# TMmichi/mujoco_jaco

Hardware: AMD Instinct MI355X
Metric: env-steps/sec at batch 65 536 (full Jaco + gripper + contacts) (higher is better)
Workload: dtype f32

## Files before the change

__graft_entry__.py:

```python
import os
import subprocess
import sys

ROOT = os.path.dirname(os.path.abspath(__file__))
CSRC = os.path.join(ROOT, "mujoco_jaco_amd", "csrc")
HIPCC = os.environ.get("HIPCC", "/opt/rocm/bin/hipcc")


D12 = ["-DJNB=13", "-DJNV=18", "-DJNQ=19", "-DJB0=12", "-DJB1=18", "-DJNSENS=64", "-DJMAXCHAIN=8", "-DJMAXDESC=12", "-DJMAXINNER=9"]
D30 = ["-DJNB=20", "-DJNV=30", "-DJNQ=32", "-DJB0=18", "-DJB1=24", "-DJNU=18", "-DJNSENS=40", "-DJMAXGEOM=128", "-DJMAXPAIR=3584", "-DJMAXINNER=12",
       "-DJMAXMPAIR=192", "-DJACO_LIGHT_WAVES=2"]


FLAGS = ["--offload-arch=gfx950", "-O3", "-std=c++17", "-fno-hip-fp32-correctly-rounded-divide-sqrt", "-fno-slp-vectorize",
         "-fgpu-flush-denormals-to-zero", "-fPIC", "-Rpass-analysis=kernel-resource-usage", "-I", os.path.join(CSRC, "include")]
NKERNEL_TU = 18


def _variant_jobs(name, extra):
    bdir = os.path.join(ROOT, "build", name)
    os.makedirs(bdir, exist_ok=True)
    jobs, objs = [], []
    for tu in list(range(NKERNEL_TU)) + [-1]:
        src = "jaco_env.hip" if tu < 0 else "kernels.hip"
# ... 15 lines not shown


def _up_to_date(cmd, log):
    obj, stamp = cmd[cmd.index("-o") + 1], log[:-4] + ".cmd"
    if not (os.path.exists(obj) and os.path.exists(stamp) and open(stamp).read() == " ".join(cmd)):
        return False
    t = os.path.getmtime(obj)
    return all(os.path.getmtime(d) < t for d in _sources_of(cmd))


def build_libs(variants, workers=None):
    workers = workers or max(1, min(8, os.cpu_count() or 1))
    todo, links = [], []
    for name, extra in variants.items():
        jobs, link = _variant_jobs(name, extra)
        jobs = [j for j in jobs if not _up_to_date(*j)]
        todo += sorted(jobs, key=lambda j: ("kernel7" in j[1], "kernel6" in j[1], "kernel5" in j[1], "kernel4" in j[1]), reverse=True)
        links.append(link)
    running, failed = [], []
    while todo or running:
        while todo and len(running) < workers and not failed:
            cmd, log = todo.pop(0)
            running.append((subprocess.Popen(cmd, cwd=CSRC, stdout=open(log, "w"), stderr=subprocess.STDOUT), cmd, log))
        if failed and not running:
            break
        p, cmd, log = running.pop(0)
        if p.poll() is None:
            running.append((p, cmd, log))
            import time
            time.sleep(0.2)
            continue
        if p.returncode == 0:
            open(log[:-4] + ".cmd", "w").write(" ".join(cmd))
        if p.returncode != 0:
            failed.append((cmd, log))
            for q, _, _ in running:
                q.terminate()
            for q, _, _ in running:
                q.wait()
            running = []
    if failed:
        cmd, log = failed[0]
        raise RuntimeError("hipcc failed: %s\n%s" % (" ".join(cmd), open(log).read()[-4000:]))
    for link in links:
        subprocess.check_call(link, cwd=CSRC)


VARIANTS = {
    "default": [],
    "d12": D12,
    "d30": D30,
    "prof": ["-DJACO_PROFILE_STAGES"],
    "noregime": ["-DJACO_NEWTON_REGIME=0"],
    "census": ["-DJACO_PROFILE_STAGES", "-DJACO_REGIME_CENSUS"],
}
PRODUCT = ("default", "d12", "d30")


def build():
    build_libs({k: v for k, v in VARIANTS.items() if k in PRODUCT or (k == "prof" and os.environ.get("JACO_BUILD_PROF") == "1")})
    subprocess.check_call(["make", "-s", "-C", os.path.join(ROOT, "oracle")])
    subprocess.check_call(["make", "-s", "-C", os.path.join(ROOT, "tests", "emu")])
    subprocess.check_call(["make", "-s", "-C", os.path.join(ROOT, "tests", "emu_lqr")])
    if os.path.isdir("/root/reference/env_script/assets/jaco2") and not os.path.exists(
            os.path.join(ROOT, "mujoco_jaco_amd", "assets", "jaco2_curtain_torque.jacomdl")):
        subprocess.check_call([sys.executable, "-m", "mujoco_jaco_amd.modelc.compile"], cwd=ROOT)
    sys.path.insert(0, ROOT)
    import mujoco_jaco_amd
    from mujoco_jaco_amd import _lib
    _lib.load()
    _lib.load("_d12")
    _lib.load("_d30")


def smoke():
    sys.path.insert(0, ROOT)
    sys.path.insert(0, os.path.join(ROOT, "tests"))
    import numpy as np
    import torch
    from mujoco_jaco_amd import workload
    from mujoco_jaco_amd.modelc import blob
    from mujoco_jaco_amd.physics import BatchedMujoco
    from oracle_binding import Oracle

    B, nsub = 64, 20
    M = blob.load(os.path.join(ROOT, "mujoco_jaco_amd", "assets", "jaco2_curtain_torque.jacomdl"))
    q = workload.reset_states(M["qpos0"], B, seed=7, f32_draws=True)
    c = workload.random_ctrl(B, seed=8, scale=0.2).astype(np.float32).astype(np.float64)
    env = BatchedMujoco(B, device=0)
    dev = env.device
    env.set_state(torch.tensor(q, dtype=torch.float32, device=dev), None, None)
    env.send_forces(torch.tensor(c, dtype=torch.float32, device=dev), nsub=nsub)
    gq, gv, _ = [t.cpu().numpy().astype(np.float64) for t in env.get_state()]
    o = Oracle()
    qo, vo, wo = q.copy(), np.zeros((B, 21)), np.zeros((B, 21))
    o.step_batch(qo, vo, wo, np.ascontiguousarray(c), nsub=nsub, nthreads=4)
    err = np.abs(gq - qo).max(axis=1)
    fl = env.flags().cpu().numpy()
    deepest = np.zeros(B)
    for k in range(B):
        o.set("qpos", q[k]); o.set("qvel", np.zeros(21)); o.forward()
        C = o.get("contact").reshape(-1, 11)
        deepest[k] = -C[:, 0].min() if len(C) else 0.0
    clean = deepest <= 0.0105
    print("smoke: %d envs x %d substeps on %s, qpos max-abs error vs fp64 oracle: median %.2e, p90 %.2e; max over the %d envs without deep start overlap %.2e, "
          "over the %d with it %.2e (deepest %.3f m); error flags %d, tiers used: %s"
# ... 16 lines not shown
```

mujoco_jaco_amd/csrc/collision.h:

```cpp
#pragma once

#define JACO_HAVE_COLLISION 1

struct GeomPose { v3 p; m3 R; };
template <class L>
JDEV GeomPose geom_pose(const L& s, int g) { GeomPose r; r.p = ld3(s.gpos[g]); r.R = ldm(s.gmat[g]); return r; }

JDEV bool obb_separated(const GeomPose& a, v3 sa, const GeomPose& b, v3 sb) {
  float C[3][3], Q[3][3];
  v3 d = b.p - a.p;
  float t[3] = {dot(d, col(a.R, 0)), dot(d, col(a.R, 1)), dot(d, col(a.R, 2))};
  float ea[3] = {sa.x, sa.y, sa.z}, eb[3] = {sb.x, sb.y, sb.z};
#pragma unroll
  for (int i = 0; i < 3; i++)
#pragma unroll
    for (int j = 0; j < 3; j++) { C[i][j] = dot(col(a.R, i), col(b.R, j)); Q[i][j] = fabsf(C[i][j]) + 1e-5f; }
  bool sep = false;
#pragma unroll
  for (int i = 0; i < 3; i++) sep |= fabsf(t[i]) > ea[i] + eb[0] * Q[i][0] + eb[1] * Q[i][1] + eb[2] * Q[i][2];
#pragma unroll
  for (int j = 0; j < 3; j++)
    sep |= fabsf(t[0] * C[0][j] + t[1] * C[1][j] + t[2] * C[2][j]) > eb[j] + ea[0] * Q[0][j] + ea[1] * Q[1][j] + ea[2] * Q[2][j];
#pragma unroll
  for (int i = 0; i < 3; i++)
// ... 884 lines not shown
      } else {
        float depth;
        v3 dir, pos;
#ifdef JACO_EMULATED
        const long q0_ = emu_counter[7];
#endif
        const MprGeom G1 = mpr_geom(m, s, g1, t1), G2 = mpr_geom(m, s, g2, t2);
#ifdef JACO_ROW_REUSE
        HullRow H1, H2;
        H1.cell = -1; H2.cell = -1; H1.e.x = H1.e.y = H1.e.z = H1.e.w = 0.f; H2.e = H1.e;
#endif
        const float sw = wave_bcast(sepA.w, c);
        bool hit = false, apart = false, sepvalid = false;
        v3 sep = mk3(0.f, 0.f, 0.f);
#if JACO_MPR_PAIRS
        if ((parked >> c) & 1ull) {
          const float* st = stash + 8 * c;
          hit = st[0] != 0.f; depth = st[1]; pos = mk3(st[2], st[3], st[4]); dir = mk3(st[5], st[6], st[7]);
          apart = true;
        } else
#endif
        if (sw != 0.f) {
          const v3 d = mk3(wave_bcast(sepA.x, c), wave_bcast(sepA.y, c), wave_bcast(sepA.z, c));
          const Sup q = mpr_support(A, G1, G2, d, lane JROWPASS);
          apart = dot(q.v, d) < -1e-5f && fabsf(dot(d, d) - 1.f) < 1e-3f;
        }
        if (!apart) {
          hit = mpr_penetration(A, m, G1, G2, lane, &depth, &dir, &pos, &sep, &sepvalid JROWPASS);
          if (seprow && lane == 0 && (sepvalid || sw != 0.f)) {
            v4 o; o.x = sep.x; o.y = sep.y; o.z = sep.z; o.w = sepvalid ? 1.f : 0.f;
            *reinterpret_cast<v4*>(seprow + 4 * pk) = o;
          }
        }
#ifdef JACO_EMULATED
        if (lane == 0 && !((parked >> c) & 1ull)) { emu_counter[3]++; emu_counter[4] += hit; emu_counter[hit ? 5 : 6] += emu_counter[7] - q0_; }
#endif
#ifdef JACO_TRACE_MPR
        if (lane == 0) printf("mpr g1 %d g2 %d hit %d depth %g\n", g1, g2, (int)hit, hit ? depth : 0.f);
#endif
        push_contacts(s, hit && lane == 0, -depth, pos, dir, pk, ncon, flags, 1);
        JSTAMP_NARROW(hit ? 14 : 1);
      }
      if (ncon > before) {
        int cc = before + lane;
        if (cc < ncon) { s.c_ob[cc] = pob; s.c_dim[cc] = pdim; }
      }
      c++;
    }
    if (L::Caps::MAXEFC < JacoHuge::MAXEFC && (wave_uniform_i((int)flags) & (int)JFLAG_CON_OVERFLOW)) break;
  }
  if (lane == 0) { s.ncon = ncon; s.ncand = ncand; }
}

#define JSIDE_ROWS 16
#define JSIDE_BASE 64
#define JSIDE_J 0
#define JSIDE_AREF 96
#define JSIDE_D 112
#define JSIDE_F 128
template <class L>
struct SideRows {
  static constexpr bool on = L::Caps::CONTACT && L::Caps::MAXEFC == 64 && JNV - JB1 == 6 && (JNV - 6) * 6 + JNB * 6 >= JSIDE_F + JSIDE_ROWS;
};
template <class L>
JDEV float* side_buf(L& s) { return &s.cdof[6][0]; }
template <class L>
JDEV float contact_row_vel(const L& s, int c, int e, float mu) {
  const int pd = s.c_dim[c];
  const int kf = pd == 1 ? 0 : 1 + (e >> 1);
  const int obs = s.c_ob[c], b1 = ((obs >> 8) & 0xFF) - 1, b2 = ((obs >> 24) & 0xFF) - 1;
  sv v1, v2;
  v1.a = v1.b = v2.a = v2.b = mk3(0.f, 0.f, 0.f);
  if (b1 >= 0) v1 = ldsv(s.cvel[b1]);
  if (b2 >= 0) v2 = ldsv(s.cvel[b2]);
  v3 cp = ld3(s.c_pos[c]);
  v3 dw = v2.a - v1.a, dv = (v2.b - v1.b) + cross(dw, cp);
  const float* fr = s.c_frame[c];
  float vel = dot(ld3(fr), dv);
  if (pd > 1) {
    const int ax = kf < 3 ? kf : kf - 3;
    const float comp = dot(ld3(fr + 3 * ax), kf < 3 ? dv : dw);
    vel += ((e & 1) ? -1.f : 1.f) * mu * comp;
  }
  return vel;
}
template <class L>
JDEV void stage_contact_rows(const JacoModelDev* m, L& s, int lane, unsigned& flags) {
  constexpr int MAXEFC = L::Caps::MAXEFC;
  constexpr bool SIDE = SideRows<L>::on;
  const int nv = m->nv, ncon = wave_uniform_i(s.ncon), nlim = wave_uniform_i(s.nlimit);
  float* sd = side_buf(s);
  int rowbase = nlim, kept_total = 0, nside = 0, side_cand = 0;
  constexpr int CPP = JNV <= 21 ? 3 : 64 / JNV;
  const int cl = lane / JNV, k = lane - cl * JNV;
  const bool dofok = cl < CPP && k < nv;
  const sv S = ldsv(s.cdof[dofok ? k : 0]);
  for (int cb = 0; cb < ncon; cb += 64) {
    const int ci = cb + lane, nhere = ncon - cb < 64 ? ncon - cb : 64;
    int dim = 0, nrow = 0;
    float mu0 = 0.f, mu1 = 0.f, mu2 = 0.f;
    unsigned cm1 = 0, cm2 = 0;
    float a0 = 0.f, bcoef = 0.f, dinv = 0.f;
    if (lane < nhere) {
      const JacoPairParam& P = m->pair[s.c_pair[ci]];
      dim = s.c_dim[ci]; nrow = dim == 1 ? 1 : 2 * (dim - 1);
      mu0 = P.mu[0]; mu1 = P.mu[2]; mu2 = P.mu[3];
      cm1 = P.m1; cm2 = P.m2;
      const float pos = s.c_dist[ci] - P.margin, tran = P.tran;
      float R, imp;
      a0 = row_params(P.solref, P.solimp, pos, 0.f, dim == 1 ? tran : tran + mu0 * mu0 * tran, &R, &imp);
      bcoef = 2.f / fmaxf(JMINVAL, fminf(0.9999f, fmaxf(0.0001f, P.solimp[1])) * P.solref[0]);
      if (dim > 1) R = fmaxf(JMINVAL, 2.f * mu0 * mu0 * R);
      dinv = 1.f / R;
    }
    const unsigned mm = cm1 | cm2;
    bool sidec = false;
    const unsigned long long upto = lane >= 63 ? ~0ull : ((2ull << lane) - 1ull);
    const unsigned long long r1m = wave_ballot(nrow == 1), r4m = wave_ballot(nrow == 4), r10m = wave_ballot(nrow == 10);
    const bool rows_std = wave_ballot(nrow != 0 && nrow != 1 && nrow != 4 && nrow != 10) == 0ull;
    int end = rowbase + (rows_std ? popc64(r1m & upto) + 4 * popc64(r4m & upto) + 10 * popc64(r10m & upto) : wave_scan_incl(nrow, lane));
#ifdef JACO_SIDE_ALWAYS
    if (JNV - JB1 == 6 && cb == 0) {
#else
    if (JNV - JB1 == 6 && cb == 0 && wave_bcast_i(end, nhere - 1) > JSIDE_BASE) {
#endif
      const bool only2 = lane < nhere && mm != 0u && (mm & ((1u << JB1) - 1u)) == 0u && nrow <= 4;
      const bool reach2 = lane < nhere && !only2 && (mm >> JB1) != 0u;
      const unsigned long long o2 = wave_ballot(only2);
      if (o2 != 0ull && wave_ballot(reach2) == 0ull && ncon <= 64) {
        int srows = 0;
        for (unsigned long long b = o2; b; b &= b - 1ull) srows += wave_bcast_i(nrow, ffs64(b));
        if (srows <= JSIDE_ROWS) { side_cand = srows; sidec = only2; }
      }
    }
    bool split = false;
    int r0s = 0;
#ifdef JACO_SIDE_ALWAYS
    if (SIDE && side_cand > 0 && wave_bcast_i(end, nhere - 1) - side_cand <= MAXEFC) {
#else
    if (SIDE && side_cand > 0 && wave_bcast_i(end, nhere - 1) > MAXEFC && wave_bcast_i(end, nhere - 1) - side_cand <= MAXEFC) {
#endif
      split = true;
      end = rowbase + wave_scan_incl(sidec ? 0 : nrow, lane);
      r0s = JSIDE_BASE + wave_scan_incl(sidec ? nrow : 0, lane) - nrow;
      nside = side_cand;
    }
    sidec = sidec && split;
    const unsigned long long fm = wave_ballot(lane < nhere && end <= MAXEFC);
    const int kept = popc64(fm);
    int total = wave_bcast_i(end, kept > 0 ? kept - 1 : 0);
    total = kept > 0 ? total : rowbase;
    const int r0 = sidec ? r0s : end - nrow;
    if (lane < kept) {
      s.c_efc[ci] = r0;
      int blk = ((mm & ((1u << JB0) - 1u)) ? 1 : 0) | (((mm >> JB0) & ((1u << (JB1 - JB0)) - 1u)) ? 2 : 0) | ((mm >> JB1) ? 4 : 0);
      const int bodies = L::Caps::WRENCH ? ((((s.c_ob[ci] >> 8) & 31) << 19) | (((s.c_ob[ci] >> 24) & 31) << 24)) : 0;
      if (!sidec) for (int e = 0; e < nrow; e++) {
        s.e_con[r0 + e] = ci | (e << 8) | (blk << 16) | bodies;
        s.e_f[r0 + e] = e < 4 ? mu0 : (e < 6 ? mu1 : mu2);
        s.e_aref[r0 + e] = a0; s.e_D[r0 + e] = dinv;
      }
      s.c_fn[ci] = bcoef;
    }
    wave_sync();
    for (int rr = rowbase + lane; rr < total; rr += 64) {
      const int ce = s.e_con[rr], c = ce & 255, e = (ce >> 8) & 255;
      const float vel = contact_row_vel(s, c, e, s.e_f[rr]);
      s.e_aref[rr] = s.e_aref[rr] - s.c_fn[c] * vel;
    }
    float aside[4] = {0.f, 0.f, 0.f, 0.f};
    if (SIDE && sidec && lane < kept) {
#pragma unroll
      for (int e = 0; e < 4; e++) if (e < nrow) aside[e] = a0 - bcoef * contact_row_vel(s, ci, e, mu0);
    }
    if (SIDE && split) {
      wave_sync();
      if (sidec && lane < kept) {
#pragma unroll
        for (int e = 0; e < 4; e++) if (e < nrow) { sd[JSIDE_AREF + r0 - JSIDE_BASE + e] = aside[e]; sd[JSIDE_D + r0 - JSIDE_BASE + e] = dinv; }
      }
    }
    if (L::Caps::WRENCH) {
      for (int rr = rowbase + lane; rr < total; rr += 64) {
        const int ce = s.e_con[rr], c = ce & 255, e = (ce >> 8) & 15, pd = s.c_dim[c];
        const int kf = pd == 1 ? 0 : 1 + (e >> 1);
        const float smu = ((e & 1) ? -1.f : 1.f) * s.e_f[rr];
        const float* fr = s.c_frame[c];
        const v3 n = ld3(fr), pos = ld3(s.c_pos[c]);
        v3 lin = n, ang = mk3(0.f, 0.f, 0.f);
        if (kf == 1 || kf == 2) lin = n + ld3(fr + 3 * kf) * smu;
        if (kf >= 3) ang = ld3(fr + 3 * (kf - 3)) * smu;
        ang = ang + cross(pos, lin);
        float* R = s.J + 8 * rr;
        R[0] = ang.x; R[1] = ang.y; R[2] = ang.z; R[3] = lin.x; R[4] = lin.y; R[5] = lin.z; R[6] = 0.f; R[7] = 0.f;
      }
    } else
    for (int c0 = 0; c0 < kept; c0 += CPP) {
      int c = c0 + (cl < CPP ? cl : 0);
      int src = c < 64 ? c : 0;
      int cdim = wave_shfl_i(dim, src), cr0 = wave_shfl_i(r0, src);
      float f0 = wave_shfl(mu0, src), f1 = wave_shfl(mu1, src), f2 = wave_shfl(mu2, src);
      unsigned a1 = (unsigned)wave_shfl_i((int)cm1, src), a2 = (unsigned)wave_shfl_i((int)cm2, src);
      const bool cside = SIDE && cr0 >= JSIDE_BASE;
      if (dofok && c < kept && (!cside || k >= JB1)) {
        float coef = (float)((int)((a2 >> k) & 1u) - (int)((a1 >> k) & 1u));
        v3 pos = ld3(s.c_pos[cb + c]);
        v3 jp = (S.b + cross(S.a, pos)) * coef, jr = S.a * coef;
        const float* fr = s.c_frame[cb + c];
        float Jc[6];
#pragma unroll
        for (int a = 0; a < 3; a++) { Jc[a] = dot(ld3(fr + 3 * a), jp); Jc[3 + a] = dot(ld3(fr + 3 * a), jr); }
        const int ld = cside ? 6 : JLD;
        float* Jw = cside ? sd + JSIDE_J + (cr0 - JSIDE_BASE) * 6 + (k - JB1) : s.J + cr0 * JLD + k;
        if (cdim == 1) Jw[0] = Jc[0];
        else {
          Jw[0] = Jc[0] + f0 * Jc[1]; Jw[ld] = Jc[0] - f0 * Jc[1];
          Jw[2 * ld] = Jc[0] + f0 * Jc[2]; Jw[3 * ld] = Jc[0] - f0 * Jc[2];
          if (cdim > 3) {
            Jw[4 * ld] = Jc[0] + f1 * Jc[3]; Jw[5 * ld] = Jc[0] - f1 * Jc[3];
            Jw[6 * ld] = Jc[0] + f2 * Jc[4]; Jw[7 * ld] = Jc[0] - f2 * Jc[4];
            Jw[8 * ld] = Jc[0] + f2 * Jc[5]; Jw[9 * ld] = Jc[0] - f2 * Jc[5];
          }
        }
      }
    }
    rowbase = total; kept_total += kept;
    if (kept < nhere) { flags |= JFLAG_EFC_OVERFLOW; break; }
  }
  const int total = rowbase;
  wave_sync();
  if (lane == 0) { s.nefc = total; s.ncon = kept_total; s.nside = nside; s.nside_cand = side_cand; }
}

JDEV bool ray_hits_site(int type, float sx, float sy, float sz, v3 p, v3 d) {
  sx += 1e-5f; sy += 1e-5f; sz += 1e-5f;
  float t0 = 0.f, t1 = 3.0e38f;
  bool ok = true;
  if (type == JG_BOX) {
    float pp[3] = {p.x, p.y, p.z}, dd[3] = {d.x, d.y, d.z}, ss[3] = {sx, sy, sz};
#pragma unroll
    for (int i = 0; i < 3; i++) {
      if (fabsf(dd[i]) < JMINVAL) { ok = ok && !(fabsf(pp[i]) > ss[i]); continue; }
      float a = (-ss[i] - pp[i]) / dd[i], b = (ss[i] - pp[i]) / dd[i];
      t0 = fmaxf(t0, fminf(a, b));
      t1 = fminf(t1, fmaxf(a, b));
    }
    return ok && t1 >= t0;
  }
  if (type == JG_CYLINDER) {
    if (fabsf(d.z) < JMINVAL) ok = !(fabsf(p.z) > sy);
    else {
      float a = (-sy - p.z) / d.z, b = (sy - p.z) / d.z;
      t0 = fmaxf(t0, fminf(a, b));
      t1 = fminf(t1, fmaxf(a, b));
    }
    float A = d.x * d.x + d.y * d.y, B = p.x * d.x + p.y * d.y, C = p.x * p.x + p.y * p.y - sx * sx;
    if (A < JMINVAL) ok = ok && !(C > 0.f);
    else {
      float disc = B * B - A * C;
      if (disc < 0.f) return false;
      float sq = sqrtf(disc);
      t0 = fmaxf(t0, (-B - sq) / A);
      t1 = fminf(t1, (-B + sq) / A);
    }
    return ok && t1 >= t0;
  }
  float A = dot(d, d), B = dot(p, d), C = dot(p, p) - sx * sx;
  if (A < JMINVAL) return C <= 0.f;
  float disc = B * B - A * C;
  if (disc < 0.f) return false;
  return (-B + sqrtf(disc)) / A >= 0.f;
}
template <class L>
JDEV void stage_touch(const JacoModelDev* m, L& s, int lane, float* sens) {
  int ncon = wave_uniform_i(s.ncon);
  {
    const unsigned sb0 = m->sens_bodymask[0], sb1 = m->sens_bodymask[1], sb2 = m->sens_bodymask[2], sb3 = m->sens_bodymask[3];
    bool mine = false;
// ... 42 lines not shown
```

mujoco_jaco_amd/csrc/physics_kernel.h:

```cpp
#pragma once
#include <stdint.h>
#include <jaco/model_dev.h>
#include <jaco/wave_ops.h>

#ifndef JACO_WRENCH
#define JACO_WRENCH 0
#endif
template <int MAXEFC_, int MAXCON_, int MAXCAND_, bool CONTACT_ = true>
struct JacoCaps {
  static_assert(MAXEFC_ % 64 == 0, "rows are dealt out 64 at a time (one per lane): the row capacity must be a multiple of 64");
  static constexpr bool WRENCH = CONTACT_ && JACO_WRENCH != 0;
  static_assert(WRENCH || JMAXGEOM != 64 || JNV != 21 || MAXCAND_ <= MAXEFC_ * 25 - 520 - 256 - 576, "default layout: the candidate list must fit behind the geom poses in the constraint-row area");
  static constexpr int MAXEFC = MAXEFC_, MAXCON = MAXCON_, MAXCAND = MAXCAND_, NR = MAXEFC_ / 64;
  static constexpr bool CONTACT = CONTACT_;
  static constexpr int JROWS = CONTACT_ ? MAXEFC_ : (JNB <= 16 ? 16 : 32), NGEOM = CONTACT_ ? JMAXGEOM : 1;
  static_assert(CONTACT_ || JNB <= 32, "limit rows of the contact-free instantiation");
};
#if JACO_WRENCH
typedef JacoCaps<128, 32, 240> JacoLight;
#else
typedef JacoCaps<64, 32, 240> JacoLight;
#endif
typedef JacoCaps<128, 32, 512> JacoMedium;
#ifndef JACO_HEAVY_ROWS
#define JACO_HEAVY_ROWS 256
#define JACO_HEAVY_CON 64
#define JACO_HEAVY_WAVES 1
#endif
typedef JacoCaps<JACO_HEAVY_ROWS, JACO_HEAVY_CON, 512> JacoHeavy;
typedef JacoCaps<64, 1, 1, false> JacoArm;
typedef JacoCaps<512, 128, 512> JacoHuge;
#define JDBG_MAXCON 64
#define JDBG_MAXEFC 256
#define JW_WT 6
#define JW_X 7
#define JW_UNIT (1 << 30)
#define JLD (JNV)

#define JFLAG_CON_OVERFLOW 1u
#define JFLAG_EFC_OVERFLOW 2u
#define JFLAG_CAND_OVERFLOW 4u
#define JFLAG_NAN 8u
#define JFLAG_SOLVER_MAXITER 16u
#define JFLAG_HEAVY_TIER 32u
#define JFLAG_BAIL_CAUSE_SHIFT 8
#define JFLAG_TIER_RETURN 128u

#define JMINVAL 1e-15f
#define JTASK_FLOATS 40

#define JPROF_N 16
struct JProfCtx {
  unsigned long long tprev;
  unsigned long long* row;
};
#ifdef JACO_PROFILE_STAGES
JDEV void jprof_stamp(JProfCtx& pc, int i, int lane) {
  unsigned long long t = __builtin_amdgcn_s_memtime();
  if (lane == 0 && pc.row) pc.row[i] += t - pc.tprev;
  pc.tprev = __builtin_amdgcn_s_memtime();
}
#define JSTAMP(i) jprof_stamp(pc, (i), lane)
#else
#define JSTAMP(i)
#endif
#ifdef JACO_NARROW_PROFILE
#define JSTAMP_NEWTON(i) JSTAMP(6)
#define JSTAMP_NARROW(i) JSTAMP(i)
#else
#define JSTAMP_NEWTON(i) JSTAMP(i)
#define JSTAMP_NARROW(i)
#endif
#ifdef JACO_REGIME_CENSUS
#undef JSTAMP
#define JSTAMP(i)
#define JCENSUS(ne, rowblocks, dual) do { if (lane == 0 && pc.row) { pc.row[0] += 1; if (((rowblocks) & 1) == 0) { pc.row[1] += 1; pc.row[2] += (dual) ? 1 : 0; pc.row[3] += (ne); } } } while (0)
#else
#define JCENSUS(ne, rowblocks, dual)
#endif

struct JacoContactRec {
  float dist, pos[3], frame[9];
  float force[6];
  int geom[2], body[2], dim;
};
#define JCONREC_WORDS 24
#define JCONREC_MAX_CAPACITY 1024
#define JSTR_(x) #x
#define JSTR(x) JSTR_(x)
static inline const char* jaco_contact_record_check(const void* rec, const int* ncon, int capacity) {
  if (!ncon || capacity < 1 || capacity > JCONREC_MAX_CAPACITY) return "needs a count buffer and 1 <= capacity <= " JSTR(JCONREC_MAX_CAPACITY);
  if ((reinterpret_cast<uintptr_t>(rec) & 15u) != 0) return "the record buffer must be 16-byte aligned";
  return nullptr;
}

enum JacoMode { JM_CTRL = 0, JM_STEP = 1, JM_FORWARD = 2, JM_HOLD = 3, JM_TAKE_ACTION = 4, JM_TERMINAL = 5, JM_PREREACH = 6 };
#define JM_REAL_STEP(m) ((m) <= JM_STEP)
#define JM_MASKED(m) ((m) == JM_FORWARD || (m) == JM_HOLD || (m) == JM_PREREACH)
#define JM_TASK_SUBSTEPS(m) ((m) == JM_STEP || (m) == JM_HOLD || (m) == JM_PREREACH)
#define JM_NO_SUBSTEP(m) ((m) == JM_TAKE_ACTION || (m) == JM_TERMINAL)

struct JacoStepArgs {
  const JacoModelDev* model;
  const float* hull;
  float* qpos;
  float* qvel;
  float* qpos_lo;
  float* qvel_lo;
  float* qacc_ws;
  const float* ctrl;
  float* sensordata;
  unsigned* flags;
  int* stats;
  int* remaining;
  struct Queue {
    int* list;
    int* count;
    int* taken;
    const int* limit;
    const int* reserve;
  } q[3];
  const int* routed_mark;
  int launch_id;
  int* light_left;
// ... 787 lines not shown
    s.e_D[r] = 1.f / R;
    s.e_con[r] = ((d < JB0 ? 1 : (d < JB1 ? 2 : 4)) << 16) | (L::Caps::WRENCH ? (JW_UNIT | (d << 19)) : 0);
  }
  if (lane == 0) { s.nefc = popc64(mask); s.nlimit = s.nefc; }
}

struct NewtonOut { float qacc, qfrc_con, qdamped; int iters; bool have_qdamped; };
#define JDAMPED_BLOCKS 1

#ifndef JACO_NEWTON_REGIME
#define JACO_NEWTON_REGIME 1
#endif
template <int NR>
JDEV void rows_dot(const float* J, const float (&jrow)[JNV], float vk, int lane, int ne, int nv, float (&out)[NR], bool free_only = false) {
  const float* Jr[NR];
#pragma unroll
  for (int q = 0; q < NR; q++) { int r = lane + 64 * q; Jr[q] = J + (r < ne ? r : 0) * JLD; out[q] = 0.f; }
  if (!(JACO_NEWTON_REGIME && free_only)) {
    float vb[JB0];
#pragma unroll
    for (int k = 0; k < JB0; k++) vb[k] = wave_bcast(vk, k);
#pragma unroll
    for (int k = 0; k < JB0; k++) {
#pragma unroll
      for (int q = 0; q < NR; q++) out[q] += (NR == 1 ? jrow[k] : Jr[q][k]) * vb[k];
    }
  }
  float vb[JNV - JB0];
#pragma unroll
  for (int k = JB0; k < JNV; k++) vb[k - JB0] = wave_bcast(vk, k);
#pragma unroll
  for (int k = JB0; k < JNV; k++) {
#pragma unroll
    for (int q = 0; q < NR; q++) out[q] += (NR == 1 ? jrow[k] : Jr[q][k]) * vb[k - JB0];
  }
  (void)nv;
}
JDEV float mat_vec(const float (&mrow)[JNV], float vk, bool free_only = false) {
  float acc = 0.f;
  if (!(JACO_NEWTON_REGIME && free_only)) {
    float vb[JB0];
#pragma unroll
    for (int k = 0; k < JB0; k++) vb[k] = wave_bcast(vk, k);
#pragma unroll
    for (int k = 0; k < JB0; k++) acc += mrow[k] * vb[k];
  }
  float vb[JNV - JB0];
#pragma unroll
  for (int k = JB0; k < JNV; k++) vb[k - JB0] = wave_bcast(vk, k);
#pragma unroll
  for (int k = JB0; k < JNV; k++) acc += mrow[k] * vb[k - JB0];
  return acc;
}
template <int NR>
JDEV float jt_vec(const float* J, const float (&f)[NR], int ne, int lane, int nv) {
  float acc = 0.f;
  int kk = lane < nv ? lane : 0;
#pragma unroll
  for (int q = 0; q < NR; q++) {
    int n = ne - 64 * q;
    n = n > 64 ? 64 : n;
    const float* Jq = J + (64 * q) * JLD + kk;
    int rl = 0;
    for (; rl + 4 <= n; rl += 4) {
      float j0 = Jq[(rl + 0) * JLD], j1 = Jq[(rl + 1) * JLD], j2 = Jq[(rl + 2) * JLD], j3 = Jq[(rl + 3) * JLD];
      const float f0 = wave_bcast(f[q], rl), f1 = wave_bcast(f[q], rl + 1), f2 = wave_bcast(f[q], rl + 2), f3 = wave_bcast(f[q], rl + 3);
      acc += j0 * f0 + j1 * f1 + j2 * f2 + j3 * f3;
    }
    for (; rl < n; rl++) acc += Jq[rl * JLD] * wave_bcast(f[q], rl);
  }
  return lane < nv ? acc : 0.f;
}

#ifndef JACO_NEWTON_LOOKAHEAD
#define JACO_NEWTON_LOOKAHEAD 1
#endif
JDEV bool newton_next_round_is_idle(bool any_row_switched, float al, float improvement, float scale, float tol) {
  const float r = 1.f - al;
  return JACO_NEWTON_LOOKAHEAD && !any_row_switched && r * r * improvement * scale < tol;
}
JDEV bool newton_qfrc_wanted(const JacoModelDev* m, const NewtonOut& out, bool dump) {
  return !JACO_NEWTON_REGIME || dump || (m->has_damping && !out.have_qdamped);
}
template <class L>
JDEV NewtonOut stage_newton(const JacoModelDev* m, L& s, const float (&mrow)[JNV], float smooth, float hd, int lane, JProfCtx& pc, bool dump) {
  (void)pc;
  constexpr int NR = L::Caps::NR, MAXEFC = L::Caps::MAXEFC;
  NewtonOut out;
  int nv = m->nv, ne = wave_uniform_i(s.nefc);
  out.qfrc_con = 0.f; out.iters = 0; out.qdamped = 0.f; out.have_qdamped = false;
  float h0[JNV];
#pragma unroll
  for (int j = 0; j < JNV; j++) h0[j] = lane < nv ? mrow[j] : (lane == j ? 1.f : 0.f);
  const int blockmask = 1 | (nv > JB0 ? 2 : 0) | (nv > JB1 ? 4 : 0);
  if (ne == 0) {
    if (m->has_damping == 1) {
      out.qacc = ldl_block0_dual(h0, smooth, hd, lane, &out.qdamped) + ldl_solve_blocks(h0, smooth, lane, blockmask & 6);
      out.have_qdamped = true;
    } else out.qacc = ldl_solve_blocks(h0, smooth, lane, blockmask);
    return out;
  }
  if (ne > MAXEFC) ne = MAXEFC;
  bool valid[NR];
  float D[NR], ar[NR], x[NR], f[NR], jp[NR];
  int blk[NR];
  float jrow[JNV];
#pragma unroll
  for (int q = 0; q < NR; q++) {
    int r = lane + 64 * q;
    valid[q] = r < ne;
    D[q] = valid[q] ? s.e_D[r] : 0.f;
    ar[q] = valid[q] ? s.e_aref[r] : 0.f;
    blk[q] = valid[q] ? (s.e_con[r] >> 16) & 7 : 0;
  }
  float scale = 1.f / (m->meaninertia * (float)(nv > 1 ? nv : 1));
  float tol = m->tolerance;
  int rowblk = 0;
#pragma unroll
  for (int q = 0; q < NR; q++) rowblk |= blk[q];
  const int rowblocks = (wave_ballot(rowblk & 1) ? 1 : 0) | (wave_ballot(rowblk & 2) ? 2 : 0) | (wave_ballot(rowblk & 4) ? 4 : 0);
  const bool mine = lane < nv && ((lane < JB0 ? 1 : (lane < JB1 ? 2 : 4)) & rowblocks) != 0;
  const bool free_only = JACO_NEWTON_REGIME && (rowblocks & 1) == 0;
#pragma unroll
  for (int k = 0; k < JNV; k++) jrow[k] = 0.f;
  if (NR == 1 && !free_only) {
#pragma unroll
    for (int k = 0; k < JB0; k++) jrow[k] = lane < ne ? s.J[lane * JLD + k] : 0.f;
  }
#pragma unroll
  for (int k = JB0; k < JNV; k++) jrow[k] = (NR == 1 && lane < ne) ? s.J[lane * JLD + k] : 0.f;
  JCENSUS(ne, rowblocks, m->has_damping == 1);
  float afree;
  if ((rowblocks & 1) == 0 && m->has_damping == 1) {
    afree = ldl_block0_dual(h0, smooth, hd, lane, &out.qdamped);
    out.have_qdamped = true;
    afree += ldl_solve_blocks(h0, smooth, lane, ~rowblocks & 6 & blockmask);
  } else afree = ldl_solve_blocks(h0, smooth, lane, ~rowblocks & 7 & blockmask);
  float a = mine ? s.qacc_ws[lane] : afree;
  float Ma = mat_vec(mrow, a, free_only) - smooth;
  Ma = mine ? Ma : 0.f;
  rows_dot<NR>(s.J, jrow, a, lane, ne, nv, x, free_only);
#pragma unroll
  for (int q = 0; q < NR; q++) x[q] = valid[q] ? x[q] - ar[q] : 0.f;
  JSTAMP_NEWTON(11);
#ifdef JACO_EMULATED
  if (lane == 0) { emu_counter[8]++; if ((rowblocks & 1) == 0) emu_counter[11]++; }
#endif
  int it = 0, nls = 0;
  for (; it < m->iterations; it++) {
    lane = wave_opaque_i(lane);
#ifdef JACO_EMULATED
    if (lane == 0) emu_counter[9]++;
#endif
    bool coupled = false;
#pragma unroll
    for (int q = 0; q < NR; q++) {
      f[q] = x[q] < 0.f ? -D[q] * x[q] : 0.f;
      coupled = coupled || (x[q] < 0.f && (blk[q] & (blk[q] - 1)) != 0);
    }
    bool full = wave_ballot(coupled) != 0ull;
    float* xs = NR == 1 ? s.smooth : s.e_x;
#pragma unroll
    for (int q = 0; q < NR; q++) if (valid[q]) { s.e_f[lane + 64 * q] = x[q] < 0.f ? D[q] : 0.f; xs[lane + 64 * q] = x[q]; }
    wave_sync();
    float h[JNV], jtf;
    if ((rowblocks & 1) == 0) {
      acc16x16 C;
      acc_zero(C);
      const int uq = lane >> 4, col = lane & 15;
      const float cj = col < JNV - JB0 ? 1.f : 0.f, cx = col == JNV - JB0 ? -1.f : 0.f;
      const float* jcol = s.J + JB0 + (col < JNV - JB0 ? col : 0);
      const int last = ne - 1;
      for (int r0 = 0; r0 < ne; r0 += 16) {
        float jv[4], wv[4];
#pragma unroll
        for (int u = 0; u < 4; u++) {
          const int r = r0 + 4 * u + uq, rc = r < last ? r : last;
          jv[u] = cj * jcol[rc * JLD] + cx * xs[rc];
          wv[u] = r < ne ? s.e_f[rc] : 0.f;
        }
#pragma unroll
        for (int u = 0; u < 4; u++) wave_mfma_16x16x4(jv[u], wv[u] * jv[u], C);
      }
      JSTAMP_NEWTON(12);
      const int jd = (lane >= JB0 && lane < JNV) ? lane - JB0 : 0;
#pragma unroll
      for (int j2 = 0; j2 < JNV; j2++) {
        float cv = 0.f;
        if (j2 >= JB0) { const int c = j2 - JB0; cv = wave_shfl(C.v[c & 3], jd + 16 * (c >> 2)); }
        h[j2] = lane < nv ? mrow[j2] + (lane >= JB0 ? cv : 0.f) : (lane == j2 ? 1.f : 0.f);
      }
      jtf = wave_shfl(C.v[(JNV - JB0) & 3], jd + 16 * ((JNV - JB0) >> 2));
      jtf = lane >= JB0 ? jtf : 0.f;
    } else {
    acc32x32 C;
    acc_zero(C);
    const int uh = lane >> 5, col = lane & 31;
    const float cj = col < JNV ? 1.f : 0.f, cx = col == JNV ? -1.f : 0.f;
    const float* jcol = s.J + (col < JNV ? col : 0);
    const int last = ne - 1;
    for (int r0 = 0; r0 < ne; r0 += 8) {
      float jv[4], wv[4];
#pragma unroll
      for (int u = 0; u < 4; u++) {
        const int r = r0 + 2 * u + uh, rc = r < last ? r : last;
        jv[u] = cj * jcol[rc * JLD] + cx * xs[rc];
        wv[u] = r < ne ? s.e_f[rc] : 0.f;
      }
#pragma unroll
      for (int u = 0; u < 4; u++) wave_mfma_32x32x2(jv[u], wv[u] * jv[u], C);
    }
    JSTAMP_NEWTON(12);
#pragma unroll
    for (int j2 = 0; j2 < JNV; j2++) {
      const int reg = (j2 & 3) + 4 * (j2 >> 3);
      float cv = ((j2 >> 2) & 1) ? wave_shfl(C.v[reg], (lane + 32) & 63) : C.v[reg];
      h[j2] = lane < nv ? mrow[j2] + cv : (lane == j2 ? 1.f : 0.f);
    }
    jtf = ((JNV >> 2) & 1) ? wave_shfl(C.v[(JNV & 3) + 4 * (JNV >> 3)], (lane + 32) & 63) : C.v[(JNV & 3) + 4 * (JNV >> 3)];
    }
    float grad = Ma - (lane < nv ? jtf : 0.f);
    float gn = sqrtf(wave_sum(grad * grad));
    if (gn * scale < tol) break;
    float p = !full ? ldl_solve_blocks(h, -grad, lane, rowblocks) : ((rowblocks & 1) == 0 ? ldl_block<JB0, JNV>(h, -grad, lane) : ldl_solve<true>(h, -grad, lane));
    p = lane < nv ? p : 0.f;
    JSTAMP_NEWTON(13);
    float Mp = mat_vec(mrow, p, free_only);
    float pMp, pMa;
    wave_sum2(p * Mp, p * Ma, &pMp, &pMa);
    rows_dot<NR>(s.J, jrow, p, lane, ne, nv, jp, free_only);
#pragma unroll
    for (int q = 0; q < NR; q++) jp[q] = valid[q] ? jp[q] : 0.f;
    float al = 0.f, lo = 0.f, hi = 3.0e38f, d10 = 0.f, dlo = 0.f, dhi = 0.f;
    for (int ls = 0; ls < m->ls_iterations; ls++) {
      float s1 = 0.f, s2 = 0.f;
#pragma unroll
      for (int q = 0; q < NR; q++) {
        float xa = x[q] + al * jp[q];
        s1 += xa < 0.f ? D[q] * xa * jp[q] : 0.f;
        s2 += xa < 0.f ? D[q] * jp[q] * jp[q] : 0.f;
      }
      float w1, w2;
      wave_sum2(s1, s2, &w1, &w2);
      float d1 = pMa + al * pMp + w1, d2 = pMp + w2;
      if (ls == 0) d10 = fabsf(d1);
#ifdef JACO_TRACE_LS
      if (lane == 0) printf("it %d ls %d al %.9g d1 %.6g d2 %.6g lo %.9g hi %.9g pMa %.6g pMp %.6g\n", it, ls, al, d1, d2, lo, hi, pMa, pMp);
#endif
      if (ls > 0 && fabsf(d1) <= 1e-6f * d10) break;
      if (d1 < 0.f) { lo = al; dlo = -d1; } else { hi = al; dhi = d1; }
      if (hi < 1.0e38f && fmaxf(dlo, dhi) * (hi - lo) * scale < 1e-3f * tol) break;
      const float stepn = d1 / d2;
      float nx = al - stepn;
      if (!(nx > lo && nx < hi)) nx = hi < 1.0e38f ? 0.5f * (lo + hi) : 2.f * al + 1.f;
      if (nx == al) break;
      al = nx;
      nls++;
    }
    float dc = 0.f;
    bool switched = false;
#pragma unroll
    for (int q = 0; q < NR; q++) {
      float dx = al * jp[q], xn = x[q] + dx;
      bool was = x[q] < 0.f, is = xn < 0.f;
      switched = switched || was != is;
      dc += (was && is) ? 0.5f * D[q] * dx * (2.f * x[q] + dx) : (is ? 0.5f * D[q] * xn * xn : (was ? -0.5f * D[q] * x[q] * x[q] : 0.f));
      x[q] = xn;
    }
    const bool any_switched = wave_ballot(switched) != 0ull;
    float improvement = -(al * pMa + 0.5f * al * al * pMp + wave_sum(dc));
    JSTAMP_NEWTON(14);
    a += al * p; Ma += al * Mp;
    if (improvement * scale < tol || newton_next_round_is_idle(any_switched, al, improvement, scale, tol)) { it++; break; }
  }
#pragma unroll
  for (int q = 0; q < NR; q++) f[q] = x[q] < 0.f ? -D[q] * x[q] : 0.f;
  out.qacc = a;
  if (newton_qfrc_wanted(m, out, dump)) out.qfrc_con = jt_vec<NR>(s.J, f, ne, lane, nv);
#ifdef JACO_EMULATED
  if (lane == 0 && newton_qfrc_wanted(m, out, dump)) emu_counter[12]++;
#endif
  out.iters = it | (nls << 8);
#pragma unroll
// ... 701 lines not shown
      if (lane >= 6 && lane < nu) s.ctrl[lane] = 0.6f;
      wave_sync();
    }
    if (emode == JM_PREREACH && phase == 1 && !held_pending) {
      if (lane >= 9 && lane < nv) { s.qvel[lane] = 0.f; s.qvel_lo[lane] = 0.f; }
      wave_sync();
    }
    if (emode == JM_STEP && !fwd) {
      if (s.task[JT_PENDING] != 0.f) {
        if (lane < nu) s.ctrl[lane] = s.task[JT_CTRL + lane];
        wave_sync();
        if (lane == 0) s.task[JT_PENDING] = 0.f;
      } else {
        stage_osc(m, s, lane, flags);
        JSTAMP(15);
        if (lane >= 6 && lane < nu) {
          float g0 = s.task[JT_GRIP_PREV], g1 = s.task[JT_GRIP];
          s.ctrl[lane] = nsub > 1 ? g0 + (g1 - g0) * ((float)sub / (float)(nsub - 1)) : g1;
        }
        wave_sync();
      }
    }
#ifdef JACO_WALK_PROFILE
    stage_walk(m, s, lane, markers, &pc);
#else
    stage_walk(m, s, lane, markers);
#endif
    for (int i = lane; i < JMBLK; i += 64) s.M[i] = 0.f;
    wave_sync();
    if constexpr (C::CONTACT) if (A.dbg && env == A.dbg_env && sub == nsub - 1 && lane < m->ngeom) for (int k = 0; k < 3; k++) A.dbg[JDBG_GPOS + 3 * lane + k] = s.gpos[lane][k];
    JSTAMP(0);
    JSTAMP(1);
    const ActParams actp = act_fetch(m, lane);
    const StagePrefetch pf = stage_prefetch(m, lane);
    stage_accumulate(m, s, lane);
    wave_sync();
    stage_mass_bias(m, s, lane, pf);
    wave_sync();
    if ((emode == JM_HOLD || (emode == JM_PREREACH && phase == 1)) && !held_pending) {
      stage_osc(m, s, lane, flags);
      if (lane >= 6 && lane < nu) s.ctrl[lane] = 0.6f;
      wave_sync();
    }
    stage_actuation(m, s, lane, actp);
    JSTAMP(2);
    unsigned cflags = 0;
    if (C::CONTACT && !A.disable_contact) {
      stage_collision(A, m, s, env, lane, cflags, pc, pl);
      wave_sync();
      JSTAMP(4);
      stage_limit_rows(m, s, lane, pf);
      wave_sync();
      JSTAMP(3);
      stage_contact_rows(m, s, lane, cflags);
      wave_sync();
      JSTAMP(5);
    } else {
      stage_limit_rows(m, s, lane, pf);
      if (lane == 0) { s.ncon = 0; s.ncand = 0; s.nsphere = 0; s.nside = 0; s.nside_cand = 0; }
      wave_sync();
    }
    if (!LIGHT) {
      constexpr int LCON = TIER == 3 ? JacoHeavy::MAXCON : (TIER == 2 ? JacoMedium::MAXCON : JacoLight::MAXCON);
      constexpr int LEFC = TIER == 3 ? JacoHeavy::MAXEFC : (TIER == 2 ? JacoMedium::MAXEFC : JacoLight::MAXEFC);
      constexpr int LCAND = TIER == 3 ? JacoHeavy::MAXCAND : (TIER == 2 ? JacoMedium::MAXCAND : JacoLight::MAXCAND);
      const bool rows_fit = s.nefc <= LEFC || (TIER == 1 && SideRows<JacoLDS<JacoLight>>::on && s.nside_cand > 0 && s.nefc - s.nside_cand <= LEFC);
      const bool fits = s.ncon <= LCON && rows_fit && s.nsphere <= LCAND;
      calm = fits ? calm + 1 : 0;
      if (!fits && !tier_used) { tier_used = true; if (A.hint_mode != 2) hint_raise(A, env, TIER, lane); }
    }
    if (TIER == 3) flags |= cflags;
    if (TIER < 3 && cflags) {
      left = nsub - sub;
      bailed = true;
      flags |= (cflags & 7u) << (JFLAG_BAIL_CAUSE_SHIFT + 3 * TIER);
      if (JM_TASK_SUBSTEPS(emode)) {
        if (lane < nu) s.task[JT_CTRL + lane] = s.ctrl[lane];
        if (lane == 0) { s.task[JT_PENDING] = 1.f; s.task[JT_SUB] = (float)sub; }
        wave_sync();
      }
      break;
    }
    float mrow[JNV], h[JNV];
    {
      const int blo = lane < JB0 ? 0 : (lane < JB1 ? JB0 : JB1), bn = lane < JB0 ? JB0 : (lane < JB1 ? JB1 - JB0 : JNV - JB1);
      const int rbase = lane < nv ? m_index(lane, blo) : 0;
#pragma unroll
      for (int j = 0; j < JNV; j++) { const bool in = lane < nv && j >= blo && j < blo + bn; mrow[j] = in ? s.M[in ? rbase + j - blo : 0] : 0.f; }
    }
    float smooth = lane < nv ? s.smooth[lane] : 0.f;
    float qas = 0.f;
    wave_sync();
    const float hdamp = (m->has_damping && lane < nv) ? m->timestep * pf.damping : 0.f;
    NewtonOut nw;
    const bool dump = A.dbg && env == A.dbg_env && sub == nsub - 1;
    if constexpr (C::WRENCH) nw = stage_newton_w(m, s, mrow, smooth, hdamp, lane, pc, dump);
    else if constexpr (C::CONTACT) nw = stage_newton(m, s, mrow, smooth, hdamp, lane, pc, dump);
    else nw = stage_newton_limits(m, s, mrow, smooth, hdamp, lane);
    if (SideRows<JacoLDS<C>>::on) { if (wave_uniform_i(s.nside) > 0) newton_side(m, s, mrow, smooth, lane, nw, dump); }
    JSTAMP(6);
    iters = nw.iters & 255;
    int nls_dbg = nw.iters >> 8;
    nls_last = nls_dbg;
    if (iters >= m->iterations) flags |= JFLAG_SOLVER_MAXITER;
    wave_sync();
    if (C::CONTACT) stage_touch(m, s, lane, &sens);
    JSTAMP(7);
// ... 516 lines not shown
```

Measured before the change: 2.069 million.

## Specialize contact Jacobian rows for free-body contacts and fuse Newton mat-vec with row dots

Adds a fast path in contact row assembly: when every kept contact touches only a 6-DoF free-body block, the wave assigns 6 lanes per contact instead of JNV lanes. It zeroes the other Jacobian columns explicitly and computes only the 6 relevant columns, which cuts the number of column-building rounds. It also fuses the Newton solver's mass-matrix mat-vec with the constraint row dot products so the broadcast vector entries are shared in a single loop. Per-stage profiling stamps and extra build variants are added for rows profiling and for disabling the free path. The costs are more code paths and extra zero-stores per row on the free path.

```diff
diff --git a/__graft_entry__.py b/__graft_entry__.py
--- a/__graft_entry__.py
+++ b/__graft_entry__.py
@@ -91,6 +91,8 @@
     "d30": D30,
     "prof": ["-DJACO_PROFILE_STAGES"],
     "noregime": ["-DJACO_NEWTON_REGIME=0"],
+    "rowsall": ["-DJACO_ROWS_FREE=0"],
+    "rowsprof": ["-DJACO_PROFILE_STAGES", "-DJACO_ROWS_PROFILE"],
     "census": ["-DJACO_PROFILE_STAGES", "-DJACO_REGIME_CENSUS"],
 }
 PRODUCT = ("default", "d12", "d30")
diff --git a/mujoco_jaco_amd/csrc/collision.h b/mujoco_jaco_amd/csrc/collision.h
--- a/mujoco_jaco_amd/csrc/collision.h
+++ b/mujoco_jaco_amd/csrc/collision.h
@@ -960,6 +960,9 @@
   if (lane == 0) { s.ncon = ncon; s.ncand = ncand; }
 }
 
+#ifndef JACO_ROWS_FREE
+#define JACO_ROWS_FREE 1
+#endif
 #define JSIDE_ROWS 16
 #define JSIDE_BASE 64
 #define JSIDE_J 0
@@ -993,9 +996,30 @@
   return vel;
 }
 template <class L>
-JDEV void stage_contact_rows(const JacoModelDev* m, L& s, int lane, unsigned& flags) {
+JDEV void contact_jac_column(const L& s, const sv S, int k, int ci, unsigned a1, unsigned a2, int cdim, float f0, float f1, float f2, float* Jw, int ld) {
+  float coef = (float)((int)((a2 >> k) & 1u) - (int)((a1 >> k) & 1u));
+  v3 pos = ld3(s.c_pos[ci]);
+  v3 jp = (S.b + cross(S.a, pos)) * coef, jr = S.a * coef;
+  const float* fr = s.c_frame[ci];
+  float Jc[6];
+#pragma unroll
+  for (int a = 0; a < 3; a++) { Jc[a] = dot(ld3(fr + 3 * a), jp); Jc[3 + a] = dot(ld3(fr + 3 * a), jr); }
+  if (cdim == 1) Jw[0] = Jc[0];
+  else {
+    Jw[0] = Jc[0] + f0 * Jc[1]; Jw[ld] = Jc[0] - f0 * Jc[1];
+    Jw[2 * ld] = Jc[0] + f0 * Jc[2]; Jw[3 * ld] = Jc[0] - f0 * Jc[2];
+    if (cdim > 3) {
+      Jw[4 * ld] = Jc[0] + f1 * Jc[3]; Jw[5 * ld] = Jc[0] - f1 * Jc[3];
+      Jw[6 * ld] = Jc[0] + f2 * Jc[4]; Jw[7 * ld] = Jc[0] - f2 * Jc[4];
+      Jw[8 * ld] = Jc[0] + f2 * Jc[5]; Jw[9 * ld] = Jc[0] - f2 * Jc[5];
+    }
+  }
+}
+template <class L>
+JDEV void stage_contact_rows(const JacoModelDev* m, L& s, int lane, unsigned& flags, JProfCtx& pc) {
   constexpr int MAXEFC = L::Caps::MAXEFC;
   constexpr bool SIDE = SideRows<L>::on;
+  (void)pc;
   const int nv = m->nv, ncon = wave_uniform_i(s.ncon), nlim = wave_uniform_i(s.nlimit);
   float* sd = side_buf(s);
   int rowbase = nlim, kept_total = 0, nside = 0, side_cand = 0;
@@ -1003,12 +1027,15 @@
   const int cl = lane / JNV, k = lane - cl * JNV;
   const bool dofok = cl < CPP && k < nv;
   const sv S = ldsv(s.cdof[dofok ? k : 0]);
+  constexpr bool FREE6 = JACO_ROWS_FREE != 0 && !L::Caps::WRENCH && JB1 - JB0 == 6 && (JNV - JB1 == 6 || JNV == JB1);
+  constexpr int CPF = 64 / 6;
   for (int cb = 0; cb < ncon; cb += 64) {
     const int ci = cb + lane, nhere = ncon - cb < 64 ? ncon - cb : 64;
     int dim = 0, nrow = 0;
     float mu0 = 0.f, mu1 = 0.f, mu2 = 0.f;
     unsigned cm1 = 0, cm2 = 0;
     float a0 = 0.f, bcoef = 0.f, dinv = 0.f;
+    JSTAMP_ROWS(5);
     if (lane < nhere) {
       const JacoPairParam& P = m->pair[s.c_pair[ci]];
       dim = s.c_dim[ci]; nrow = dim == 1 ? 1 : 2 * (dim - 1);
@@ -1021,6 +1048,7 @@
       if (dim > 1) R = fmaxf(JMINVAL, 2.f * mu0 * mu0 * R);
       dinv = 1.f / R;
     }
+    JSTAMP_ROWS(11);
     const unsigned mm = cm1 | cm2;
     bool sidec = false;
     const unsigned long long upto = lane >= 63 ? ~0ull : ((2ull << lane) - 1ull);
@@ -1059,9 +1087,11 @@
     int total = wave_bcast_i(end, kept > 0 ? kept - 1 : 0);
     total = kept > 0 ? total : rowbase;
     const int r0 = sidec ? r0s : end - nrow;
+    const int blk = ((mm & ((1u << JB0) - 1u)) ? 1 : 0) | (((mm >> JB0) & ((1u << (JB1 - JB0)) - 1u)) ? 2 : 0) | ((mm >> JB1) ? 4 : 0);
+    const bool freec = FREE6 && !split && kept > 0 && wave_ballot(lane < kept && blk != 2 && blk != 4) == 0ull;
+    JSTAMP_ROWS(12);
     if (lane < kept) {
       s.c_efc[ci] = r0;
-      int blk = ((mm & ((1u << JB0) - 1u)) ? 1 : 0) | (((mm >> JB0) & ((1u << (JB1 - JB0)) - 1u)) ? 2 : 0) | ((mm >> JB1) ? 4 : 0);
       const int bodies = L::Caps::WRENCH ? ((((s.c_ob[ci] >> 8) & 31) << 19) | (((s.c_ob[ci] >> 24) & 31) << 24)) : 0;
       if (!sidec) for (int e = 0; e < nrow; e++) {
         s.e_con[r0 + e] = ci | (e << 8) | (blk << 16) | bodies;
@@ -1071,10 +1101,21 @@
       s.c_fn[ci] = bcoef;
     }
     wave_sync();
+    JSTAMP_ROWS(13);
     for (int rr = rowbase + lane; rr < total; rr += 64) {
       const int ce = s.e_con[rr], c = ce & 255, e = (ce >> 8) & 255;
       const float vel = contact_row_vel(s, c, e, s.e_f[rr]);
       s.e_aref[rr] = s.e_aref[rr] - s.c_fn[c] * vel;
+      if (freec) {
+        float* Jz = s.J + rr * JLD;
+#pragma unroll
+        for (int a = 0; a < JB0; a++) Jz[a] = 0.f;
+        if (JNV - JB1 == 6) {
+          Jz += ((ce >> 16) & 2) ? JB1 : JB0;
+#pragma unroll
+          for (int a = 0; a < 6; a++) Jz[a] = 0.f;
+        }
+      }
     }
     float aside[4] = {0.f, 0.f, 0.f, 0.f};
     if (SIDE && sidec && lane < kept) {
@@ -1088,6 +1129,7 @@
         for (int e = 0; e < 4; e++) if (e < nrow) { sd[JSIDE_AREF + r0 - JSIDE_BASE + e] = aside[e]; sd[JSIDE_D + r0 - JSIDE_BASE + e] = dinv; }
       }
     }
+    JSTAMP_ROWS(14);
     if (L::Caps::WRENCH) {
       for (int rr = rowbase + lane; rr < total; rr += 64) {
         const int ce = s.e_con[rr], c = ce & 255, e = (ce >> 8) & 15, pd = s.c_dim[c];
@@ -1103,35 +1145,34 @@
         R[0] = ang.x; R[1] = ang.y; R[2] = ang.z; R[3] = lin.x; R[4] = lin.y; R[5] = lin.z; R[6] = 0.f; R[7] = 0.f;
       }
     } else
+    if (freec) {
+      const int cf = lane / 6, kf = lane - cf * 6;
+      for (int c0 = 0; c0 < kept; c0 += CPF) {
+#ifdef JACO_EMULATED
+        if (lane == 0) emu_counter[14]++;
+#endif
+        const int c = c0 + (cf < CPF ? cf : 0), src = c < 64 ? c : 0;
+        const int cdim = wave_shfl_i(dim, src), cr0 = wave_shfl_i(r0, src);
+        const float f0 = wave_shfl(mu0, src), f1 = wave_shfl(mu1, src), f2 = wave_shfl(mu2, src);
+        const unsigned a1 = (unsigned)wave_shfl_i((int)cm1, src), a2 = (unsigned)wave_shfl_i((int)cm2, src);
+        const int kk = (((a1 | a2) >> JB1) ? JB1 : JB0) + kf;
+        if (cf < CPF && c < kept && kk < nv) contact_jac_column(s, ldsv(s.cdof[kk]), kk, cb + c, a1, a2, cdim, f0, f1, f2, s.J + cr0 * JLD + kk, JLD);
+      }
+    } else
     for (int c0 = 0; c0 < kept; c0 += CPP) {
+#ifdef JACO_EMULATED
+      if (lane == 0) emu_counter[15]++;
+#endif
       int c = c0 + (cl < CPP ? cl : 0);
       int src = c < 64 ? c : 0;
       int cdim = wave_shfl_i(dim, src), cr0 = wave_shfl_i(r0, src);
       float f0 = wave_shfl(mu0, src), f1 = wave_shfl(mu1, src), f2 = wave_shfl(mu2, src);
       unsigned a1 = (unsigned)wave_shfl_i((int)cm1, src), a2 = (unsigned)wave_shfl_i((int)cm2, src);
       const bool cside = SIDE && cr0 >= JSIDE_BASE;
-      if (dofok && c < kept && (!cside || k >= JB1)) {
-        float coef = (float)((int)((a2 >> k) & 1u) - (int)((a1 >> k) & 1u));
-        v3 pos = ld3(s.c_pos[cb + c]);
-        v3 jp = (S.b + cross(S.a, pos)) * coef, jr = S.a * coef;
-        const float* fr = s.c_frame[cb + c];
-        float Jc[6];
-#pragma unroll
-        for (int a = 0; a < 3; a++) { Jc[a] = dot(ld3(fr + 3 * a), jp); Jc[3 + a] = dot(ld3(fr + 3 * a), jr); }
-        const int ld = cside ? 6 : JLD;
-        float* Jw = cside ? sd + JSIDE_J + (cr0 - JSIDE_BASE) * 6 + (k - JB1) : s.J + cr0 * JLD + k;
-        if (cdim == 1) Jw[0] = Jc[0];
-        else {
-          Jw[0] = Jc[0] + f0 * Jc[1]; Jw[ld] = Jc[0] - f0 * Jc[1];
-          Jw[2 * ld] = Jc[0] + f0 * Jc[2]; Jw[3 * ld] = Jc[0] - f0 * Jc[2];
-          if (cdim > 3) {
-            Jw[4 * ld] = Jc[0] + f1 * Jc[3]; Jw[5 * ld] = Jc[0] - f1 * Jc[3];
-            Jw[6 * ld] = Jc[0] + f2 * Jc[4]; Jw[7 * ld] = Jc[0] - f2 * Jc[4];
-            Jw[8 * ld] = Jc[0] + f2 * Jc[5]; Jw[9 * ld] = Jc[0] - f2 * Jc[5];
-          }
-        }
-      }
-    }
+      if (dofok && c < kept && (!cside || k >= JB1))
+        contact_jac_column(s, S, k, cb + c, a1, a2, cdim, f0, f1, f2, cside ? sd + JSIDE_J + (cr0 - JSIDE_BASE) * 6 + (k - JB1) : s.J + cr0 * JLD + k, cside ? 6 : JLD);
+    }
+    JSTAMP_ROWS(1);
     rowbase = total; kept_total += kept;
     if (kept < nhere) { flags |= JFLAG_EFC_OVERFLOW; break; }
   }
diff --git a/mujoco_jaco_amd/csrc/physics_kernel.h b/mujoco_jaco_amd/csrc/physics_kernel.h
--- a/mujoco_jaco_amd/csrc/physics_kernel.h
+++ b/mujoco_jaco_amd/csrc/physics_kernel.h
@@ -64,12 +64,20 @@
 #else
 #define JSTAMP(i)
 #endif
+#if defined(JACO_NARROW_PROFILE) || defined(JACO_ROWS_PROFILE)
+#define JSTAMP_NEWTON(i) JSTAMP(6)
+#else
+#define JSTAMP_NEWTON(i) JSTAMP(i)
+#endif
 #ifdef JACO_NARROW_PROFILE
-#define JSTAMP_NEWTON(i) JSTAMP(6)
 #define JSTAMP_NARROW(i) JSTAMP(i)
 #else
-#define JSTAMP_NEWTON(i) JSTAMP(i)
 #define JSTAMP_NARROW(i)
+#endif
+#if defined(JACO_ROWS_PROFILE) && defined(JACO_PROFILE_STAGES) && !defined(JACO_EMULATED)
+#define JSTAMP_ROWS(i) do { __builtin_amdgcn_sched_barrier(0); __builtin_amdgcn_s_waitcnt(0); JSTAMP(i); __builtin_amdgcn_sched_barrier(0); } while (0)
+#else
+#define JSTAMP_ROWS(i)
 #endif
 #ifdef JACO_REGIME_CENSUS
 #undef JSTAMP
@@ -963,6 +971,44 @@
   for (int k = JB0; k < JNV; k++) acc += mrow[k] * vb[k - JB0];
   return acc;
 }
+#ifndef JACO_NEWTON_FUSE
+#define JACO_NEWTON_FUSE 1
+#endif
+template <int NR>
+JDEV float mat_vec_rows_dot(const float (&mrow)[JNV], const float* J, const float (&jrow)[JNV], float vk, int lane, int ne, int nv, float (&out)[NR], bool free_only) {
+#if JACO_NEWTON_FUSE
+  const float* Jr[NR];
+#pragma unroll
+  for (int q = 0; q < NR; q++) { int r = lane + 64 * q; Jr[q] = J + (r < ne ? r : 0) * JLD; out[q] = 0.f; }
+  float acc = 0.f;
+  if (!(JACO_NEWTON_REGIME && free_only)) {
+    float vb[JB0];
+#pragma unroll
+    for (int k = 0; k < JB0; k++) vb[k] = wave_bcast(vk, k);
+#pragma unroll
+    for (int k = 0; k < JB0; k++) {
+      acc += mrow[k] * vb[k];
+#pragma unroll
+      for (int q = 0; q < NR; q++) out[q] += (NR == 1 ? jrow[k] : Jr[q][k]) * vb[k];
+    }
+  }
+  float vb[JNV - JB0];
+#pragma unroll
+  for (int k = JB0; k < JNV; k++) vb[k - JB0] = wave_bcast(vk, k);
+#pragma unroll
+  for (int k = JB0; k < JNV; k++) {
+    acc += mrow[k] * vb[k - JB0];
+#pragma unroll
+    for (int q = 0; q < NR; q++) out[q] += (NR == 1 ? jrow[k] : Jr[q][k]) * vb[k - JB0];
+  }
+  (void)nv;
+  return acc;
+#else
+  const float acc = mat_vec(mrow, vk, free_only);
+  rows_dot<NR>(J, jrow, vk, lane, ne, nv, out, free_only);
+  return acc;
+#endif
+}
 template <int NR>
 JDEV float jt_vec(const float* J, const float (&f)[NR], int ne, int lane, int nv) {
   float acc = 0.f;
@@ -1048,9 +1094,8 @@
     afree += ldl_solve_blocks(h0, smooth, lane, ~rowblocks & 6 & blockmask);
   } else afree = ldl_solve_blocks(h0, smooth, lane, ~rowblocks & 7 & blockmask);
   float a = mine ? s.qacc_ws[lane] : afree;
-  float Ma = mat_vec(mrow, a, free_only) - smooth;
+  float Ma = mat_vec_rows_dot<NR>(mrow, s.J, jrow, a, lane, ne, nv, x, free_only) - smooth;
   Ma = mine ? Ma : 0.f;
-  rows_dot<NR>(s.J, jrow, a, lane, ne, nv, x, free_only);
 #pragma unroll
   for (int q = 0; q < NR; q++) x[q] = valid[q] ? x[q] - ar[q] : 0.f;
   JSTAMP_NEWTON(11);
@@ -1136,10 +1181,9 @@
     float p = !full ? ldl_solve_blocks(h, -grad, lane, rowblocks) : ((rowblocks & 1) == 0 ? ldl_block<JB0, JNV>(h, -grad, lane) : ldl_solve<true>(h, -grad, lane));
     p = lane < nv ? p : 0.f;
     JSTAMP_NEWTON(13);
-    float Mp = mat_vec(mrow, p, free_only);
+    float Mp = mat_vec_rows_dot<NR>(mrow, s.J, jrow, p, lane, ne, nv, jp, free_only);
     float pMp, pMa;
     wave_sum2(p * Mp, p * Ma, &pMp, &pMa);
-    rows_dot<NR>(s.J, jrow, p, lane, ne, nv, jp, free_only);
 #pragma unroll
     for (int q = 0; q < NR; q++) jp[q] = valid[q] ? jp[q] : 0.f;
     float al = 0.f, lo = 0.f, hi = 3.0e38f, d10 = 0.f, dlo = 0.f, dhi = 0.f;
@@ -1947,7 +1991,7 @@
       stage_limit_rows(m, s, lane, pf);
       wave_sync();
       JSTAMP(3);
-      stage_contact_rows(m, s, lane, cflags);
+      stage_contact_rows(m, s, lane, cflags, pc);
       wave_sync();
       JSTAMP(5);
     } else {
```

New measurement: 2.118 million (median of 6 runs). 1.02x the previous value.
